# mikwieczorek/centroids-reid

Hardware: AMD Instinct MI355X
Metric: train_images_per_sec (higher is better)
Workload: dtype bf16; 1 GPU; ResNet50 256x128 CTL training step: fwd+bwd, centroid-triplet + center + xent, Adam + center SGD (BASELINE configs[1]); P=16, K=4, global_batch=64, num_classes=751, parallelism=single

## Files before the change

### centroids-reid_amd/_lib.py

```python
from __future__ import annotations

import ctypes as C
import os

import torch

_HERE = os.path.dirname(os.path.abspath(__file__))
LIB_PATH = os.environ.get("CREID_LIB_PATH") or os.path.join(_HERE, "lib", "libcreid_hip.so")

F32, BF16, F16 = 0, 1, 2
_DT = {torch.float32: F32, torch.bfloat16: BF16, torch.float16: F16}
BF16X3 = 3
EVAL_PRECISIONS = ("bf16x3",)
TRAIN_PRECISIONS = ("bf16x3",)

_lib = None

_p, _i64, _i32, _f32, _sz = C.c_void_p, C.c_int64, C.c_int32, C.c_float, C.c_size_t

SIGNATURES = {
    "creid_abi_version": (C.c_int, []),
    "creid_l2norm_rows": (C.c_int, [_p, _p, _p, _i64, _i64, C.c_int, _f32, _p]),
    "creid_row_sqnorm": (C.c_int, [_p, _p, _i64, _i64, C.c_int, _p]),
    "creid_sqdist_matrix": (C.c_int, [_p, _p, _p, _p, _i64, _i64, _i64, C.c_int, _p, _i64, _p]),
# ... 18 lines not shown
    "creid_stream_count_band_h16": (C.c_int, [_p, _p, _p, _p, _i64, _i64, _i64, C.c_int, _p, _p, _i32, _p, _p, _p, _p, _i32, _p, _p, _p,
                                              _p]),
    "creid_stream_count_rescore": (C.c_int, [_p, _p, _i64, _i32, _p, _p, _p, _p, _i64, _i64, _i32, _p, _p, _p, _p, _p, _p]),
    "creid_rerank_recip": (C.c_int, [_p, _i64, _i32, _i32, _p, _p, _p, _p]),
    "creid_rerank_weights": (C.c_int, [_p, _p, _p, _i64, _i64, _p, _p, _p, _p]),
    "creid_rerank_expand": (C.c_int, [_p, _i64, _i32, _i32, _p, _p, _p, _i32, _p, _p, _p, _p, _p]),
    "creid_rerank_blend": (C.c_int, [_p, _p, _i64, _i64, _f32, _p, _p, _p, _p, _p, _i32, _p, _p]),
    "creid_tune_set": (C.c_int, [_i32, _i64, _i64, _i64, _i64, _i32, _i32, _i32]),
    "creid_tune_clear": (C.c_int, []),
    "creid_tune_count": (_i64, [_i32, _i64, _i64, _i64, _i64, _i32]),
    "creid_loo_centroids_fwd": (C.c_int, [_p, _p, _i64, _i64, _i64, _p, _p, _p]),
    "creid_loo_centroids_bwd": (C.c_int, [_p, _p, _i64, _i64, _i64, _p, _p]),
    "creid_loo_emb_fwd": (C.c_int, [_p, _p, _p, _i64, _i64, _i64, _p, _p, _p, _p, _p, _p]),
    "creid_loo_emb_bwd": (C.c_int, [_p, _p, _i64, _i64, _i64, _p, _p]),
    "creid_ctl_step_stats": (C.c_int, [_p, _p, _i64, _i64, _p, _i64, _p, _p]),
    "creid_loo_emb_fwd_rows": (C.c_int, [_p, _p, _p, _i64, _i64, _i64, _p, _p, _p, _p, _p, _p, _p]),
    "creid_loo_emb_fwd_rows_lonely": (C.c_int, [_p, _p, _p, _i64, _i64, _i64, _p, _p, _p, _p, _p, _p, _p, _p]),
    "creid_triplet_fwd_batched_rows": (C.c_int, [_p, _p, _p, _i64, _i64, _i64, _f32, _i32, _p, _p, _p, _p, _p, _p, _p]),
    "creid_ctl_round_scale": (C.c_int, [_p, _i64, _p, _p]),
    "creid_ctl_heads_workspace_bytes": (_sz, [_i64, _i64, _i64, _i64, _i64]),
    "creid_ctl_heads_fused": (C.c_int, [_p, _p]),
    "creid_ctl_step_stats_rows": (C.c_int, [_p, _p, _i64, _i64, _i64, _p, _p, _p, _p]),
    "creid_center_loss_fwd_masked": (C.c_int, [_p, _p, _p, _p, _i64, _i64, _i64, _p, _p, _p]),
    "creid_center_loss_bwd_masked": (C.c_int, [_p, _p, _p, _p, _p, _i64, _i64, _p, _f32, _p, _p, _p]),
    "creid_xent_ls_masked": (C.c_int, [_p, _p, _p, _i64, _i64, _f32, _f32, _p, _p, _p, _p]),
    "creid_bn1d_fwd_masked": (C.c_int, [_p, _p, _i64, _i64, _p, _p, _p, _p, _f32, _f32, _p, _p, _p, _p]),
    "creid_bn1d_bwd_masked": (C.c_int, [_p, _p, _p, _i64, _i64, _p, _p, _p, _p, _p, _p, _p]),
    "creid_triplet_fwd": (C.c_int, [_p, _p, _p, _i64, _i64, _f32, _p, _p, _p, _p, _p, _p, _p, _p]),
    "creid_triplet_bwd": (C.c_int, [_p, _i64, _i64, _p, _p, _p, _p, _p, _p, _f32, _p, _p]),
    "creid_triplet_fwd_batched": (C.c_int, [_p, _p, _p, _i64, _i64, _i64, _f32, _p, _p, _p, _p, _p, _p, _p, _p]),
    "creid_triplet_bwd_batched": (C.c_int, [_p, _i64, _i64, _i64, _p, _p, _p, _p, _p, _p, _f32, _p, _p]),
    "creid_triplet_cosine_fwd": (C.c_int, [_p, _p, _p, _i64, _i64, _f32, _p, _p, _p, _p, _p, _p, _p, _p]),
    "creid_triplet_cosine_bwd": (C.c_int, [_p, _i64, _i64, _p, _p, _p, _p, _p, _p, _f32, _p, _p]),
    "creid_rownorm_fwd": (C.c_int, [_p, _i64, _i64, C.c_int, _f32, _p, _p, _p]),
    "creid_rownorm_bwd": (C.c_int, [_p, _p, _p, _i64, _i64, C.c_int, _f32, _p, _p]),
    "creid_hard_mine_from_dist": (C.c_int, [_p, _p, _i64, _p, _p, _p, _p, _p]),
    "creid_clamp_sqrt_inplace": (C.c_int, [_p, _i64, _f32, _p]),
    "creid_center_loss_fwd": (C.c_int, [_p, _p, _p, _i64, _i64, _i64, _p, _p, _p]),
    "creid_center_loss_bwd": (C.c_int, [_p, _p, _p, _p, _i64, _i64, _p, _f32, _p, _p, _p]),
    "creid_xent_ls": (C.c_int, [_p, _p, _i64, _i64, _f32, _f32, _p, _p, _p, _p]),
    "creid_bn1d_fwd": (C.c_int, [_p, _i64, _i64, _p, _p, _p, _p, C.c_int, _f32, _f32, _p, _p, _p, _p]),
    "creid_bn1d_bwd": (C.c_int, [_p, _p, _i64, _i64, _p, _p, _p, _p, _p, _p, _p]),
    "creid_gather_mean_rows": (C.c_int, [_p, _p, _p, _i64, _i64, _p, _p]),
    "creid_adam_step": (C.c_int, [_p, _p, _p, _p, _i64, _f32, _f32, _f32, _f32, _f32, _i64, _f32, _p]),
    "creid_adam_step_dev": (C.c_int, [_p, _p, _p, _p, _i64, _p, _f32, _f32, _f32, _f32, _f32, _p]),
    "creid_sgd_scaled_step": (C.c_int, [_p, _p, _i64, _f32, _f32, _p]),
    "creid_amp_scale": (C.c_int, [_p, _i64, _p, _p, _p]),
    "creid_amp_unscale_check": (C.c_int, [_p, _i64, _p, _p, _p]),
    "creid_amp_update": (C.c_int, [_p, _p, _f32, _f32, C.c_int32, _p]),
    "creid_adam_step_dev_amp": (C.c_int, [_p, _p, _p, _p, _i64, _p, _f32, _f32, _f32, _f32, _f32, _p, _p]),
    "creid_sgd_scaled_step_amp": (C.c_int, [_p, _p, _i64, _f32, _f32, _p, _p]),
    "creid_conv2d_bn_partial_rows": (_i64, [_p]),
    "creid_igemm_halo_launches": (_i64, []),
    "creid_wgrad_taps_launches": (_i64, []),
    "creid_conv2d_fwd_nhwc": (C.c_int, [_p, _p, _p, _p, _p, C.c_int, _p]),
    "creid_conv2d_fwd_affine_nhwc": (C.c_int, [_p, _p, _p, _p, _p, _p, C.c_int, C.c_int, _p]),
    "creid_conv1x1_bnrelu_fwd": (C.c_int, [_p, _p, _p, _i64, _i64, _i64, _p, _p, _p, _p, C.c_int, _p]),
    "creid_bn2d_fold_entry_bytes": (_i64, []),
    "creid_bn2d_fold_multi": (C.c_int, [_p, _i64, _p]),
    "creid_stem_conv_fwd_affine": (C.c_int, [_i64, _i64, _i64, _p, _p, _p, _p, C.c_int, C.c_int, _p]),
    "creid_stem_conv_pool_fwd_affine": (C.c_int, [_i64, _i64, _i64, _p, _p, _p, _p, C.c_int, C.c_int, _p]),
    "creid_bottleneck_c3_c1_fwd_affine": (C.c_int, [_i64, _i64, _i64, _i64, _p, _p, _p, _p, _p, _p, _p, _p, C.c_int, _p]),
    "creid_bottleneck_c3_c1_fwd_stats": (C.c_int, [_i64, _i64, _i64, _i64, _p, _p, _p, _p, _p, _p, _p, _p, C.c_int, _p]),
    "creid_conv2d_dgrad_nhwc": (C.c_int, [_p, _p, _p, _p, _p, C.c_int, _p]),
    "creid_conv2d_wgrad_workspace_bytes": (_sz, [_p, C.c_int]),
    "creid_conv2d_wgrad_nhwc": (C.c_int, [_p, _p, _p, _p, C.c_int, _p, _sz, C.c_int, _p]),
    "creid_conv2d_wgrad_partials": (C.c_int, [_p, _p, _p, _p, _sz, C.c_int, _p]),
    "creid_conv2d_wgrad_partials_bnfin": (C.c_int, [_p, _p, _p, _p, _sz, C.c_int, _p, _i64, _i64, _i64, _p, _p, _p, _p, _p, _p, _p]),
    "creid_conv2d_wgrad_reduce": (C.c_int, [_p, _p, C.c_int, _p, _sz, C.c_int, _p]),
    "creid_bn2d_bwd_finalize_wred": (C.c_int, [_p, _i64, _i64, _i64, _p, _p, _p, _p, _p, _p, _p, _p, C.c_int, _p, _sz, C.c_int, _p]),
    "creid_conv2d_wgrad_reduce_job": (C.c_int, [_p, _p, C.c_int, _p, _sz, C.c_int, _p]),
    "creid_conv2d_dgrad_x3_nhwc": (C.c_int, [_p, _p, _p, _p, _p, _p]),
    "creid_conv2d_wgrad_x3_workspace_bytes": (_sz, [_p]),
    "creid_conv2d_wgrad_x3_nhwc": (C.c_int, [_p, _p, _p, _p, C.c_int, _p, _sz, _p]),
    "creid_conv2d_wgrad_x3_partials": (C.c_int, [_p, _p, _p, _p, _sz, _p]),
    "creid_weight_prep_x3_train_multi": (C.c_int, [_p, _p, _i64, _i64, _p]),
    "creid_stem_conv_fwd": (C.c_int, [_i64, _i64, _i64, _p, _p, _p, _p, C.c_int, _p]),
    "creid_stem_conv_wgrad_workspace_bytes": (_sz, [_i64, _i64, _i64, C.c_int]),
    "creid_stem_conv_wgrad": (C.c_int, [_i64, _i64, _i64, _p, _p, _p, C.c_int, _p, _sz, C.c_int, _p]),
    "creid_image_to_nhwc4_pad": (C.c_int, [_p, _i64, _i64, _i64, C.c_int, _p, _p]),
    "creid_augment_u8": (C.c_int, [_p, _p, _i64, _i64, _i64, _i64] + [C.c_float] * 9 + [C.c_int32, C.c_int32, _p, _p]),
    "creid_resize_u8": (C.c_int, [_p, _i64, _p, _p, _p, _i64, _p, _i64, _i64, _i64, _p, _p]),
    "creid_weight_prep": (C.c_int, [_p, _i64, _i64, _i64, _i64, C.c_int, _p, _p, _p]),
    "creid_weight_prep_entry_bytes": (_i64, []),
    "creid_weight_prep_multi": (C.c_int, [_p, _p, _i64, _i64, C.c_int, _p]),
    "creid_stem_weight_prep": (C.c_int, [_p, C.c_int, _p, _p]),
    "creid_bn2d_finalize": (C.c_int, [_p, _i64, _i64, _i64, _p, _p, C.c_int, _f32, _f32, _p, _p, _p, _p, _p, _p]),
    "creid_col_stats_rows": (_i64, [_i64]),
    "creid_col_stats": (C.c_int, [_p, _i64, _i64, C.c_int, _p, _p]),
    "creid_bn2d_apply": (C.c_int, [_p, _p, _p, C.c_int, _i64, _i64, C.c_int, _p, _p]),
    "creid_bn2d_apply_mask": (C.c_int, [_p, _p, _p, C.c_int, _i64, _i64, C.c_int, _p, _p, _p]),
    "creid_bn2d_finalize_apply_mask": (C.c_int, [_p, _i64, _i64, _i64, _p, _p, _f32, _f32, _p, _p, _p, _p, _p, _p, _p, C.c_int, C.c_int, _p, _p, C.c_int, _p]),
    "creid_bn2d_apply_dual_mask": (C.c_int, [_p, _p, _p, _p, C.c_int, _i64, _i64, C.c_int, _p, _p, _p]),
    "creid_bn2d_bwd_rows": (_i64, [_i64]),
    "creid_bn2d_bwd": (C.c_int, [_p, _p, _p, _p, _p, _p, _i64, _i64, C.c_int, _p, C.c_int, _p, _p, _p, _p, _p, _p]),
    "creid_bn2d_bwd_mask": (C.c_int, [_p, _p, _p, _p, _p, _p, _p, _i64, _i64, C.c_int, _p, C.c_int, _p, _p, _p, _p, _p, _p]),
    "creid_bn2d_bwd_mask_reduce2": (C.c_int, [_p, _p, _p, _p, _p, _p, _i64, _i64, C.c_int, _p, C.c_int, _p, _p, _p, _p, _p, _p, _p, _p, _p]),
    "creid_conv2d_dgrad_bnred_nhwc": (C.c_int, [_p, _p, _p, _p, _p, _p, _p, _p, _p, _p, _i64, C.c_int, C.c_int, _p]),
    "creid_conv2d_dgrad_fused_nhwc": (C.c_int, [_p, _p, _p, _p, _p, C.c_int, _p, _p, _p, _p, _p, _p, _p, _i64, _p, _p, C.c_int, _p, _sz,
                                                C.c_int, _p]),
    "creid_ibn_rows_per_image": (_i64, [_i64]),
    "creid_ibn_fwd": (C.c_int, [_p, _i64, _i64, _i64, _i64, _p, _p, _p, _p, _p, _p, C.c_int, _f32, _f32, C.c_int, C.c_int,
                                _p, C.c_int, _p, _p, _p, _p, _p]),
    "creid_ibn_bwd": (C.c_int, [_p, _p, _p, _p, _p, _i64, _i64, _i64, _i64, _p, _p, C.c_int, _p, C.c_int, _p, _p, _p, _p, _p,
                                _p, _p, _p]),
    "creid_ibn_fwd_mask": (C.c_int, [_p, _i64, _i64, _i64, _i64, _p, _p, _p, _p, _p, _p, C.c_int, _f32, _f32, C.c_int, C.c_int, _p, C.c_int, _p, _p, _p, _p, _p, _p]),
# ... 106 lines not shown
```

### centroids-reid_amd/csrc/conv_igemm.hip

```cpp
#include "conv_epilogue.hpp"
#include <type_traits>
#include <atomic>
#include "wgrad_reduce.hpp"
#include "tune.hpp"
#include <stdlib.h>

bool wgrad_make_reduce_job(const creid_conv_desc* d, int dtype, const void* ws, size_t ws_bytes, float* dw, int accumulate,
                           WRedJob& j);
int wgrad_reduce_job_launch(const WRedJob& j, hipStream_t s);
int launch_stream1x1(int M, int K, int N, const void* src, const void* wgt, void* out, float* bn_part, hipStream_t s);
int launch_stream2(int M, int K, int N, const void* src, const void* wgt, void* out, float* bn_part, const void* add_src,
                   const float* epi_scale, const float* epi_shift, int epi_relu, int bn_cap, int dtype, hipStream_t s);
int launch_conv3x3_c64(int M, int H, int Wd, const void* src, const void* wgt, void* out, float* bn_part, const float* epi_scale,
                       const float* epi_shift, int epi_relu, int dtype, hipStream_t s);
int launch_igemm_pp(const IGemmGeom& g, const void* src, const void* wgt, void* out, const void* add_src, float* bn_part,
                    int variant, int dtype, hipStream_t s);

__device__ __attribute__((aligned(128))) unsigned g_zero_page[32];

template <int BN>
__global__ __launch_bounds__(256, BN == 128 ? 1 : 2) void igemm_bf16_kernel(IGemmGeom g, const unsigned short* __restrict__ src,
                                                         const unsigned short* __restrict__ wgt,
                                                         unsigned short* __restrict__ out,
                                                         const unsigned short* __restrict__ add_src,
// ... 811 lines not shown
    for (int tap = 0; tap < 9; ++tap) {
      const int dr = g.transposed ? 2 - tr : tr, dc = g.transposed ? 2 - ts : ts;
      int aoff[MI], kx[MI];
#pragma unroll
      for (int i = 0; i < MI; ++i) {
        const int hr = hr0[i] + dr, hc = hc0[i] + dc;
        aoff[i] = (hr * hp + hc) * BK;
        kx[i] = (((hc >> 1) + kmul * hr) & 7) ^ kh;
      }
      if (++ts == 3) { ts = 0; ++tr; }
#pragma unroll
      for (int kc = 0; kc < P; ++kc) {
        asm volatile("s_barrier" ::: "memory");
        const unsigned short* As = smem + kc * PLANE;
        const unsigned short* Bs = smem + HALO + buf * TILE_B;
        buf = (buf + 1 == NS) ? 0 : buf + 1;
        s16x8 a[2][MI], b[2][TNW];
        auto load_frags = [&](int kk, int sl) {
          const int ch = 2 * kk + kh;
#pragma unroll
          for (int i = 0; i < MI; ++i)
            a[sl][i] = *reinterpret_cast<const s16x8*>(&As[aoff[i] + (((2 * kk) ^ kx[i]) << 3)]);
#pragma unroll
          for (int j = 0; j < TNW; ++j) {
            const int c = wn * (BN / 2) + j * 32 + l31;
            b[sl][j] = *reinterpret_cast<const s16x8*>(&Bs[c * BK + ((ch ^ ((c >> 1) & 7)) << 3)]);
          }
        };
        auto mma = [&](int sl) {
          if (CREID_ABL_ON(g.abl, 1)) return;
#pragma unroll
          for (int i = 0; i < MI; ++i)
#pragma unroll
            for (int j = 0; j < TNW; ++j)
              acc[i][j] = ET::mfma(a[sl][i], b[sl][j], acc[i][j]);
        };
        load_frags(0, 0);
        __builtin_amdgcn_sched_barrier(0);
        load_frags(1, 1); mma(0);
        __builtin_amdgcn_sched_barrier(0);
        load_frags(2, 0); mma(1);
        __builtin_amdgcn_sched_barrier(0);
        load_frags(3, 1); mma(0);
        __builtin_amdgcn_sched_barrier(0);
        mma(1);
      }
    }
  }
  __syncthreads();

  igemm_tile_epilogue<ET, BM, BN, NT>(g, smem, acc, out, add_src, bn_part, bnred, tile_m, row0, col0, [](int rr) { return rr; });
}

template <int BN>
__global__ __launch_bounds__(256) void igemm_f32_kernel(IGemmGeom g, const float* __restrict__ src,
                                                        const float* __restrict__ wgt, float* __restrict__ out,
                                                        const float* __restrict__ add_src,
                                                        float* __restrict__ bn_part, int tiles_n) {
  constexpr int BK = 16, PA = 128 * 4 + 16, PB = BN * 4 + 16, TNW = BN / 64, NB = BN / 64;
  __shared__ __attribute__((aligned(16))) float As[2][2][2][PA];
  __shared__ __attribute__((aligned(16))) float Bs[2][2][2][PB];
  const int tid = threadIdx.x, lane = tid & 63, wave = tid >> 6;
  const int wm = wave >> 1, wn = wave & 1;
  const int bid = xcd_remap(blockIdx.x, gridDim.x);
  const int tile_m = bid / tiles_n, tile_n = bid % tiles_n;
  const int row0 = tile_m * 128, col0 = tile_n * BN;
  const int span_mask = (1 << g.log2span) - 1;

  const int lrow = tid >> 2, lkc = tid & 3;
  int oy[2], ox[2], bpix[2];
  bool vm[2];
#pragma unroll
  for (int i = 0; i < 2; ++i) {
    const int m = row0 + lrow + 64 * i;
    vm[i] = m < g.M;
    const int mm = vm[i] ? m : 0;
    const int b = mm / (g.OH * g.OW), rem = mm - b * (g.OH * g.OW);
    oy[i] = rem / g.OW; ox[i] = rem - oy[i] * g.OW;
    bpix[i] = b * g.SH * g.SW;
  }
  const float* wp[NB];
#pragma unroll
  for (int i = 0; i < NB; ++i) wp[i] = wgt + (int64_t)(col0 + lrow + 64 * i) * g.K + 4 * lkc;
  float4 ra[2], rb[NB];
  unsigned amask[2] = {0u, 0u};
  auto gload = [&](int t) {
    const int kk = t * BK + 4 * lkc;
    const int tap = kk >> g.log2span, c = kk & span_mask;
    const int r = tap / g.kw, s = tap - r * g.kw;
#pragma unroll
    for (int i = 0; i < 2; ++i) {
      int iy, ix;
      const bool ok = vm[i] && igemm_src_pixel(g, oy[i], ox[i], r, s, iy, ix);
      amask[i] = ok ? 0xffffffffu : 0u;
      const int64_t off = ok ? (int64_t)(bpix[i] + iy * g.SW + ix) * g.pitch + c : 0;
      ra[i] = *reinterpret_cast<const float4*>(src + off);
    }
#pragma unroll
    for (int i = 0; i < NB; ++i) rb[i] = *reinterpret_cast<const float4*>(wp[i] + t * BK);
  };
  const int sh = lkc >> 1, so = lrow * 4 + 2 * (lkc & 1);
  auto lstore = [&](int buf) {
#pragma unroll
    for (int i = 0; i < 2; ++i) {
      auto mk = [&](float v) { return __uint_as_float(__float_as_uint(v) & amask[i]); };
      *reinterpret_cast<float2*>(&As[buf][0][sh][so + 256 * i]) = make_float2(mk(ra[i].x), mk(ra[i].z));
// ... 77 lines not shown
    float s1 = 0.f, s2 = 0.f;
    const float esc = g.epi_scale ? g.epi_scale[c] : 1.f, esh = g.epi_scale ? g.epi_shift[c] : 0.f;
#pragma unroll
    for (int i = 0; i < 2; ++i) {
#pragma unroll
      for (int r = 0; r < 16; ++r) {
        const int rr = row0 + wm * 64 + i * 32 + (r & 3) + 8 * (r >> 2) + 4 * kh;
        if (rr < g.M) {
          float v = acc[i][j][r];
          if (g.epi_scale) v = fmaf(v, esc, esh);
          if (add_src) v += add_src[(int64_t)rr * g.N + c];
          if (g.epi_relu) v = fmaxf(v, 0.f);
          s1 += v; s2 = fmaf(v, v, s2);
          out[(int64_t)rr * g.N + c] = v;
        }
      }
    }
    if (bn_part) {
      s1 += __shfl_xor(s1, 32, 64); s2 += __shfl_xor(s2, 32, 64);
      if (kh == 0) { red[(wm * 2 + 0) * BN + cl] = s1; red[(wm * 2 + 1) * BN + cl] = s2; }
    }
  }
  if (bn_part) {
    __syncthreads();
    for (int i = tid; i < 2 * BN; i += 256) {
      const int which = i / BN, cl = i - which * BN;
      bn_part[((int64_t)tile_m * 2 + which) * g.N + col0 + cl] = red[(0 * 2 + which) * BN + cl] + red[(1 * 2 + which) * BN + cl];
    }
  }
}

static int use_dma_env() {
  static const int v = [] { const char* e = getenv("CREID_IGEMM_DMA"); return e ? atoi(e) : 1; }();
  return v;
}

static int ws_stages_env() {
  static const int v = [] { const char* e = getenv("CREID_IGEMM_WS_STAGES"); int x = e ? atoi(e) : 0; return (x == 2 || x == 4) ? x : 3; }();
  return v;
}

static bool igemm_halo_covers(const IGemmGeom& g, int bn, int stages) {
  const int c = 1 << g.log2span;
  if (g.kw != 3 || g.K != 9 * c || g.stride != 1 || g.pad != 1 || !g.check_bounds || g.parity || g.pitch != c) return false;
  if (c != 64 && c != 128 && c != 256) return false;
  if (g.SH != g.OH || g.SW != g.OW) return false;
  if (g.OW != 8 && g.OW != 16 && g.OW != 32 && g.OW != 64) return false;
  if ((g.OH * g.OW) % 128 != 0 || g.M % (g.OH * g.OW) != 0) return false;
  if ((128 / g.OW + 2) * (g.OW + 2) > 32 * halo_pw(c)) return false;
  if (stages < 2 || stages > 4 || (bn != 64 && bn != 128)) return false;
  return halo_lds_bytes(c, bn, stages) < 160 * 1024;
}
static std::atomic<long long> g_halo_launches{0};

static int launch_igemm(const IGemmGeom& g_in, const void* src, const void* wgt, void* out, const void* add_src,
                        float* bn_part, int dtype, hipStream_t s, BnRedArgs bnred = BnRedArgs{},
                        const WRedJob* wred_in = nullptr) {
#ifdef CREID_ABL_BUILD
  const char* abl_e = CREID_KNOB_ENV("CREID_IGEMM_ABL");
  const int abl_env = abl_e ? atoi(abl_e) : 0;
  { static int warned = -1; if (abl_env && abl_env != warned) { warned = abl_env; creid_ablation_env("CREID_IGEMM_ABL"); } }
#else
  const int abl_env = 0;
#endif
  if (!creid_is_storage(dtype)) return CREID_E_DTYPE;
  IGemmGeom g = g_in;
  g.abl = abl_env;
  WRedJob wred{};
  if (wred_in) wred = *wred_in;
  static_assert(sizeof(float) * (4 * 512 + 8192) <= 2 * (128 + 64) * 64 * 2, "reduce scratch must fit the smallest LDS ring");
  const int tiles_m = (g.M + 127) / 128;
  int bn = 128;
  static const int min_wgs = [] { const char* e = getenv("CREID_IGEMM_BN128_MIN_WGS"); int v = e ? atoi(e) : 0; return v > 0 ? v : 384; }();
  if (g.N % 128 != 0 || (int64_t)tiles_m * (g.N / 128) < min_wgs) bn = 64;
  TunePlan tp;
  int tuned_stages = 0, tuned_dma = 0, tuned_stream = 0, tuned_bm256 = 0, tuned_stream2 = 0, tuned_pp = -1;
  const int plan_d = g.transposed | (g.stride << 1);
  const bool plan_eval = creid_is16(dtype) && g.epi_scale && creid_tune_lookup(CREID_TUNE_IGEMM, g.M, g.N, g.K, plan_d | 8, tp);
  const bool have_plan = plan_eval || (creid_is16(dtype) && creid_tune_lookup(CREID_TUNE_IGEMM, g.M, g.N, g.K, plan_d, tp));
  int planned = -1;
  auto ran = [&](int kernel) {
    if (have_plan && kernel != planned) creid_tune_declined(CREID_TUNE_IGEMM, g.M, g.N, g.K, plan_eval ? (plan_d | 8) : plan_d);
  };
  if (have_plan && dtype == CREID_F16 && tp.p2 == 2) {
  } else if (have_plan && tp.p2 == 5) {
    tuned_pp = tp.p0;
    planned = 5;
  } else if (have_plan && (tp.p0 == 64 || tp.p0 == 128) && g.N % tp.p0 == 0 && (tp.p1 == 2 || tp.p1 == 3 || tp.p1 == 4)) {
    bn = tp.p0; tuned_stages = tp.p1; tuned_dma = tp.p2 == 1; tuned_stream = tp.p2 == 2; tuned_bm256 = tp.p2 == 3; tuned_stream2 = tp.p2 == 4;
    planned = (tp.p2 >= 1 && tp.p2 <= 4) ? tp.p2 : 0;
  }
  {
    const char* ce = CREID_KNOB_ENV("CREID_C64_3X3");
    const bool c64_on = !ce || atoi(ce) != 0;
    if (c64_on && creid_is16(dtype) && !g.transposed && g.N == 64 && g.K == 576 && g.log2span == 6 && g.kw == 3 && g.stride == 1 &&
        g.pad == 1 && g.pitch == 64 && g.check_bounds && !add_src && !bnred.x && !wred.ws && g.SH == g.OH && g.SW == g.OW &&
        !(bn_part && g.epi_scale)) {
      const int rc = launch_conv3x3_c64(g.M, g.OH, g.OW, src, wgt, out, bn_part, g.epi_scale, g.epi_shift, g.epi_relu, dtype, s);
      if (rc != CREID_E_SHAPE) { ran(6); return rc; }
    }
  }
  {
    const char* pe = CREID_KNOB_ENV("CREID_IGEMM_PP");
    const int force_pp = pe ? (int)strtol(pe, nullptr, 0) : 0;
    const bool pp_off = pe && force_pp == 0;
    if (creid_is16(dtype) && !bnred.x && !wred.ws && g.log2span >= 6 && !pp_off && (force_pp || tuned_pp >= 0)) {
// ... 36 lines not shown
      static const int parity_on = [] { const char* e = getenv("CREID_DGRAD_PARITY"); return e ? atoi(e) : 1; }();
      IGemmGeom gp = g;
      if (parity_on && g.transposed && g.stride == 2 && g.kw == 3 && g.pad == 1 && (g.K >> g.log2span) == 9 &&
          g.OH % 2 == 0 && g.OW % 2 == 0 && (g.M / 4) % 128 == 0 && !g.add_compact && bnred.tiles_per_image == 0)
        gp.parity = 1;
      int ws_stages = use_ws == 2 ? ws_stages_env() : ((bn == 64 && g.K >= ws_min_k) ? 3 : 2);
      if (tuned_stages && use_ws != 2) ws_stages = tuned_stages;
      const dim3 block_ws(512);
      {
        const char* be = CREID_KNOB_ENV("CREID_IGEMM_BM");
        const int force_bm = be ? atoi(be) : 0;
        static const int bm256_min = [] { const char* e = getenv("CREID_IGEMM_BM256_MIN_WGS"); int v = e ? atoi(e) : 0; return v > 0 ? v : 256; }();
        const bool can256 = g.N % 128 == 0 && !bnred.x && !gp.parity;
        const int64_t wgs256 = (int64_t)((g.M + 255) / 256) * (g.N / 128);
        if (can256 && force_bm != 128 && (tuned_bm256 || (force_bm == 256 && wgs256 >= bm256_min))) {
          const int st256 = (ws_stages >= 3 || g.K >= 256) ? 3 : 2;
          const dim3 grid256((unsigned)(wgs256 + (wred.ws ? wred.nblocks : 0)));
          const int tn256 = g.N / 128;
#define CREID_WS256_LAUNCH(NS_, ET_)                                                                                  \
  hipLaunchKernelGGL((igemm_bf16_ws_kernel<128, NS_, 256, ET_>), grid256, block_ws, 0, s, gp, (const unsigned short*)src, \
                     (const unsigned short*)wgt, (unsigned short*)out, (const unsigned short*)add_src, bn_part, tn256, bnred, wred)
          if (dtype == CREID_F16) { if (st256 == 3) CREID_WS256_LAUNCH(3, F16T); else CREID_WS256_LAUNCH(2, F16T); }
          else { if (st256 == 3) CREID_WS256_LAUNCH(3, Bf16T); else CREID_WS256_LAUNCH(2, Bf16T); }
#undef CREID_WS256_LAUNCH
          ran(tuned_bm256 ? 3 : -2);
          return (int)hipGetLastError();
        }
      }
      if (ws_stages == 4 && bn == 128 && !(tuned_stages == 4 && use_ws != 2)) ws_stages = 3;
      const dim3 grid_ws((unsigned)(tiles_m * tiles_n + (wred.ws ? wred.nblocks : 0)));
      {
        const char* he = CREID_KNOB_ENV("CREID_IGEMM_HALO");
        if ((!he || atoi(he) != 0) && igemm_halo_covers(gp, bn, ws_stages)) {
          const int hc = 1 << gp.log2span;
#define CREID_HALO_LAUNCH1(C_, BN_, NS_, ET_)                                                                             \
  hipLaunchKernelGGL((igemm_bf16_halo_kernel<C_, BN_, NS_, ET_>), grid_ws, block_ws, 0, s, gp, (const unsigned short*)src, \
                     (const unsigned short*)wgt, (unsigned short*)out, (const unsigned short*)add_src, bn_part, tiles_n,  \
                     bnred, wred)
#define CREID_HALO_LAUNCH(C_, BN_, NS_) do { if (dtype == CREID_F16) CREID_HALO_LAUNCH1(C_, BN_, NS_, F16T); else CREID_HALO_LAUNCH1(C_, BN_, NS_, Bf16T); } while (0)
#define CREID_HALO_STAGES(C_, BN_) do { constexpr int NS4 = halo_lds_bytes(C_, BN_, 4) < 160 * 1024 ? 4 : 3;            \
                                        if (ws_stages == 4) CREID_HALO_LAUNCH(C_, BN_, NS4);                            \
                                        else if (ws_stages == 2) CREID_HALO_LAUNCH(C_, BN_, 2); else CREID_HALO_LAUNCH(C_, BN_, 3); } while (0)
#define CREID_HALO_BN(C_) do { if (bn == 128) CREID_HALO_STAGES(C_, 128); else CREID_HALO_STAGES(C_, 64); } while (0)
          if (hc == 64) CREID_HALO_BN(64); else if (hc == 128) CREID_HALO_BN(128); else CREID_HALO_BN(256);
#undef CREID_HALO_BN
#undef CREID_HALO_STAGES
#undef CREID_HALO_LAUNCH
#undef CREID_HALO_LAUNCH1
          g_halo_launches.fetch_add(1, std::memory_order_relaxed);
          ran(0);
          return (int)hipGetLastError();
        }
      }
#define CREID_WS_LAUNCH1(BN_, NS_, ET_)                                                                               \
  hipLaunchKernelGGL((igemm_bf16_ws_kernel<BN_, NS_, 128, ET_>), grid_ws, block_ws, 0, s, gp, (const unsigned short*)src, \
                     (const unsigned short*)wgt, (unsigned short*)out, (const unsigned short*)add_src, bn_part, tiles_n, \
                     bnred, wred)
#define CREID_WS_LAUNCH(BN_, NS_) do { if (dtype == CREID_F16) CREID_WS_LAUNCH1(BN_, NS_, F16T); else CREID_WS_LAUNCH1(BN_, NS_, Bf16T); } while (0)
      if (bn == 128) { if (ws_stages == 4) CREID_WS_LAUNCH(128, 4); else if (ws_stages == 2) CREID_WS_LAUNCH(128, 2); else CREID_WS_LAUNCH(128, 3); }
      else { if (ws_stages == 4) CREID_WS_LAUNCH(64, 4); else if (ws_stages == 2) CREID_WS_LAUNCH(64, 2); else CREID_WS_LAUNCH(64, 3); }
#undef CREID_WS_LAUNCH
#undef CREID_WS_LAUNCH1
      ran(0);
      return (int)hipGetLastError();
    }
    if (wred.ws) { const int rc = wgrad_reduce_job_launch(wred, s); if (rc) return rc; wred.ws = nullptr; }
    static const int stages_env = [] { const char* e = getenv("CREID_IGEMM_STAGES"); int v = e ? atoi(e) : 0; return (v >= 2 && v <= 5) ? v : 2; }();
    const int stages = (tuned_dma && tuned_stages) ? tuned_stages : stages_env;
#define CREID_DMA_LAUNCH1(BN_, NS_, ET_)                                                                               \
  hipLaunchKernelGGL((igemm_bf16_dma_kernel<BN_, NS_, ET_>), grid, block, 0, s, g, (const unsigned short*)src,         \
                     (const unsigned short*)wgt, (unsigned short*)out, (const unsigned short*)add_src, bn_part, tiles_n, \
                     bnred)
#define CREID_DMA_LAUNCH(BN_, NS_) do { if (dtype == CREID_F16) CREID_DMA_LAUNCH1(BN_, NS_, F16T); else CREID_DMA_LAUNCH1(BN_, NS_, Bf16T); } while (0)
    if (bn == 128) {
      switch (stages) { case 2: CREID_DMA_LAUNCH(128, 2); break; case 3: CREID_DMA_LAUNCH(128, 3); break;
                        case 4: case 5: CREID_DMA_LAUNCH(128, 4); break;
                        default: CREID_DMA_LAUNCH(128, 2); break; }
    } else {
      switch (stages) { case 2: CREID_DMA_LAUNCH(64, 2); break; case 3: CREID_DMA_LAUNCH(64, 3); break;
                        case 4: CREID_DMA_LAUNCH(64, 4); break; case 5: CREID_DMA_LAUNCH(64, 5); break;
                        default: CREID_DMA_LAUNCH(64, 2); break; }
    }
#undef CREID_DMA_LAUNCH
#undef CREID_DMA_LAUNCH1
    ran(1);
    return (int)hipGetLastError();
  } else if (bnred.x || g.add_mask || (g.epi_scale && creid_is16(dtype)) || dtype == CREID_F16) {
    return CREID_E_DTYPE;
  } else if (wred.ws && wgrad_reduce_job_launch(wred, s) != 0) {
    return (int)hipGetLastError();
  } else if (dtype == CREID_BF16) {
    if (g.K % 64 != 0) return CREID_E_SHAPE;
    if (bn == 128)
      hipLaunchKernelGGL(igemm_bf16_kernel<128>, grid, block, 0, s, g, (const unsigned short*)src,
                         (const unsigned short*)wgt, (unsigned short*)out, (const unsigned short*)add_src, bn_part, tiles_n);
    else
      hipLaunchKernelGGL(igemm_bf16_kernel<64>, grid, block, 0, s, g, (const unsigned short*)src,
                         (const unsigned short*)wgt, (unsigned short*)out, (const unsigned short*)add_src, bn_part, tiles_n);
  } else if (dtype == CREID_F32) {
    if (g.K % 16 != 0) return CREID_E_SHAPE;
    if (bn == 128)
      hipLaunchKernelGGL(igemm_f32_kernel<128>, grid, block, 0, s, g, (const float*)src, (const float*)wgt, (float*)out,
                         (const float*)add_src, bn_part, tiles_n);
    else
      hipLaunchKernelGGL(igemm_f32_kernel<64>, grid, block, 0, s, g, (const float*)src, (const float*)wgt, (float*)out,
                         (const float*)add_src, bn_part, tiles_n);
  } else {
    return CREID_E_DTYPE;
  }
  ran(-2);
  return (int)hipGetLastError();
}

static int check_desc(const creid_conv_desc* d) {
  if (!d || d->batch <= 0 || d->in_h <= 0 || d->in_w <= 0 || d->in_c <= 0 || d->out_c <= 0) return CREID_E_ARG;
  if (d->kh != d->kw || (d->kh != 1 && d->kh != 3) || d->stride < 1 || d->stride > 2) return CREID_E_SHAPE;
  if (igemm_ilog2(d->in_c) < 0 || igemm_ilog2(d->out_c) < 0 || d->in_c < 64 || d->out_c < 64) return CREID_E_SHAPE;
  if (d->out_h != (d->in_h + 2 * d->pad - d->kh) / d->stride + 1) return CREID_E_SHAPE;
  if (d->out_w != (d->in_w + 2 * d->pad - d->kw) / d->stride + 1) return CREID_E_SHAPE;
  if (d->batch * d->in_h * d->in_w >= (1LL << 24) || d->batch * d->out_h * d->out_w >= (1LL << 24) || d->batch * d->in_h * d->in_w * d->in_c > (1LL << 40)) return CREID_E_SHAPE;
  return 0;
}

int conv_check_desc(const creid_conv_desc* d) { return check_desc(d); }

extern "C" {

int64_t creid_igemm_halo_launches(void) { return (int64_t)g_halo_launches.load(std::memory_order_relaxed); }

int64_t creid_conv2d_bn_partial_rows(const creid_conv_desc* d) {
  if (!d) return 0;
  return (d->batch * d->out_h * d->out_w + 127) / 128;
}

int creid_conv2d_fwd_nhwc(const creid_conv_desc* d, const void* x, const void* w_krsc, void* y, float* bn_partial,
                          int dtype, void* stream) {
  int rc = check_desc(d);
  if (rc) return rc;
  CREID_CHECK_ARG(x && w_krsc && y);
  IGemmGeom g = fwd_geom(d);
  if (dtype == CREID_BF16X3) return launch_igemm_x3(g, x, w_krsc, y, nullptr, bn_partial, as_stream(stream));
  return launch_igemm(g, x, w_krsc, y, nullptr, bn_partial, dtype, as_stream(stream));
}

int creid_conv2d_fwd_affine_nhwc(const creid_conv_desc* d, const void* x, const void* w_krsc, void* y, const float* scale_shift,
                                 const void* residual, int relu, int dtype, void* stream) {
  int rc = check_desc(d);
  if (rc) return rc;
  CREID_CHECK_ARG(x && w_krsc && y && scale_shift);
  IGemmGeom g = fwd_geom(d);
  g.epi_scale = scale_shift; g.epi_shift = scale_shift + d->out_c; g.epi_relu = relu ? 1 : 0;
  if (dtype == CREID_BF16X3) return launch_igemm_x3(g, x, w_krsc, y, residual, nullptr, as_stream(stream));
  return launch_igemm(g, x, w_krsc, y, residual, nullptr, dtype, as_stream(stream));
}

int creid_conv2d_dgrad_nhwc(const creid_conv_desc* d, const void* dy, const void* w_crsk, void* dx, const void* add_src,
                            int dtype, void* stream) {
  int rc = check_desc(d);
  if (rc) return rc;
  CREID_CHECK_ARG(dy && w_crsk && dx);
  IGemmGeom g = dgrad_geom(d);
  return launch_igemm(g, dy, w_crsk, dx, add_src, nullptr, dtype, as_stream(stream));
}

int creid_conv2d_dgrad_x3_nhwc(const creid_conv_desc* d, const void* dy, const void* w2_crsk, void* dx, const void* add_src,
                               void* stream) {
  int rc = check_desc(d);
  if (rc) return rc;
  CREID_CHECK_ARG(dy && w2_crsk && dx);
  IGemmGeom g = dgrad_geom(d);
  return launch_igemm_x3(g, dy, w2_crsk, dx, add_src, nullptr, as_stream(stream));
}

int creid_conv2d_dgrad_bnred_nhwc(const creid_conv_desc* d, const void* dy, const void* w_crsk, void* dx,
                                  const void* add_src, const void* bn_x, const void* bn_act, const float* bn_mean,
                                  const float* bn_invstd, float* bn_partial, int64_t bn_stat_image_rows,
                                  int add_src_stride, int dtype, void* stream) {
  int rc = check_desc(d);
  if (rc) return rc;
  CREID_CHECK_ARG(dy && w_crsk && dx && bn_x && bn_mean && bn_invstd && bn_partial && bn_stat_image_rows >= 0);
  return creid_conv2d_dgrad_fused_nhwc(d, dy, w_crsk, dx, add_src, add_src_stride, nullptr, bn_x, bn_act, nullptr, bn_mean, bn_invstd,
// ... 53 lines not shown
```

### include/creid.h

```cpp
#ifndef CREID_H
#define CREID_H

#include <stddef.h>
#include <stdint.h>

#ifdef __cplusplus
extern "C" {
#endif

#define CREID_ABI_VERSION 1

enum { CREID_F32 = 0, CREID_BF16 = 1, CREID_F16 = 2, CREID_BF16X3 = 3 };
enum { CREID_E_ARG = -1, CREID_E_DTYPE = -2, CREID_E_WS = -3, CREID_E_SHAPE = -4 };

int creid_abi_version(void);


int creid_l2norm_rows(const float* x, void* y, float* sqnorm, int64_t rows, int64_t D,
                      int out_dtype, float eps, void* stream);

int creid_row_sqnorm(const void* x, float* out, int64_t rows, int64_t D, int dtype, void* stream);

int creid_sqdist_matrix(const void* q, const void* g, const float* qq, const float* gg,
                        int64_t m, int64_t n, int64_t D, int dtype, float* out, int64_t ldo,
// ... 192 lines not shown
                              float* dist_an, int32_t* p_idx, int32_t* n_idx, void* stream);

int creid_clamp_sqrt_inplace(float* d, int64_t n, float lo, void* stream);

int creid_center_loss_fwd(const float* x, const int64_t* labels, const float* centers, int64_t B,
                          int64_t C, int64_t D, float* row_sq, float* loss, void* stream);
int creid_center_loss_bwd(const float* x, const int64_t* labels, const float* centers,
                          const float* row_sq, int64_t B, int64_t D, const float* gscale_dev,
                          float gscale, float* dx_accum, float* dcenters_accum, void* stream);

int creid_xent_ls(const float* logits, const int64_t* targets, int64_t B, int64_t C, float eps,
                  float gscale, float* row_loss, float* loss, float* dlogits, void* stream);

int creid_bn1d_fwd(const float* x, int64_t B, int64_t D, const float* weight, const float* bias,
                   float* running_mean, float* running_var, int training, float momentum, float eps,
                   float* y, float* save_mean, float* save_invstd, void* stream);
int creid_bn1d_bwd(const float* x, const float* dy, int64_t B, int64_t D, const float* weight,
                   const float* save_mean, const float* save_invstd, float* dx_accum,
                   float* dweight_accum, float* dbias_accum, void* stream);

int creid_gather_mean_rows(const float* emb, const int64_t* order, const int64_t* offsets,
                           int64_t n_seg, int64_t D, float* out, void* stream);


int creid_adam_step(float* p, const float* g, float* m, float* v, int64_t n, float lr, float beta1,
                    float beta2, float eps, float weight_decay, int64_t step, float grad_scale,
                    void* stream);
int creid_adam_step_dev(float* p, const float* g, float* m, float* v, int64_t n, float* hyper_dev,
                        float beta1, float beta2, float eps, float weight_decay, float grad_scale,
                        void* stream);
int creid_sgd_scaled_step(float* p, float* g, int64_t n, float lr, float grad_mul, void* stream);

int creid_amp_scale(const float* x, int64_t n, const float* amp_state, float* y, void* stream);
int creid_amp_unscale_check(float* g, int64_t n, const float* amp_state, int32_t* amp_flags, void* stream);
int creid_amp_update(float* amp_state, int32_t* amp_flags, float growth_factor, float backoff_factor, int32_t growth_interval,
                     void* stream);
int creid_adam_step_dev_amp(float* p, const float* g, float* m, float* v, int64_t n, float* hyper_dev, float beta1, float beta2,
                            float eps, float weight_decay, float grad_scale, const int32_t* skip_flag, void* stream);
int creid_sgd_scaled_step_amp(float* p, float* g, int64_t n, float lr, float grad_mul, const int32_t* skip_flag, void* stream);


int creid_gemm_f32(const float* A, int64_t sam, int64_t sak, const float* B, int64_t sbk, int64_t sbn,
                   float* C, int64_t ldc, int64_t M, int64_t N, int64_t K, float alpha, float beta,
                   int32_t split_k, void* stream);


typedef struct {
  int64_t batch, in_h, in_w, in_c, out_h, out_w, out_c;
  int32_t kh, kw, stride, pad;
} creid_conv_desc;

int64_t creid_conv2d_bn_partial_rows(const creid_conv_desc* d);
int64_t creid_igemm_halo_launches(void);
int64_t creid_wgrad_taps_launches(void);
int creid_conv2d_fwd_nhwc(const creid_conv_desc* d, const void* x, const void* w_krsc, void* y,
                          float* bn_partial, int dtype, void* stream);
int creid_conv2d_fwd_affine_nhwc(const creid_conv_desc* d, const void* x, const void* w_krsc, void* y,
                                 const float* scale_shift, const void* residual, int relu, int dtype, void* stream);
int creid_conv1x1_bnrelu_fwd(const void* x_raw, const float* scale_shift, const void* w_krsc, int64_t M, int64_t K, int64_t N,
                             void* y, float* bn_partial, void* a_out, uint8_t* mask_out, int dtype, void* stream);
int64_t creid_bn2d_fold_entry_bytes(void);
int creid_bn2d_fold_multi(const void* table_dev, int64_t n_entries, void* stream);
int creid_conv2d_dgrad_nhwc(const creid_conv_desc* d, const void* dy, const void* w_crsk, void* dx,
                            const void* add_src, int dtype, void* stream);
int creid_conv2d_dgrad_x3_nhwc(const creid_conv_desc* d, const void* dy, const void* w2_crsk, void* dx, const void* add_src,
                               void* stream);
int creid_conv2d_dgrad_bnred_nhwc(const creid_conv_desc* d, const void* dy, const void* w_crsk, void* dx,
                                  const void* add_src, const void* bn_x, const void* bn_act,
                                  const float* bn_mean, const float* bn_invstd, float* bn_partial,
                                  int64_t bn_stat_image_rows, int add_src_stride, int dtype, void* stream);

int creid_conv2d_dgrad_fused_nhwc(const creid_conv_desc* d, const void* dy, const void* w_crsk, void* dx,
                                  const void* add_src, int add_src_stride, const uint8_t* add_mask, const void* bn_x,
                                  const void* bn_act, const uint8_t* bn_mask, const float* bn_mean, const float* bn_invstd,
                                  float* bn_partial, int64_t bn_stat_image_rows, const creid_conv_desc* wred_desc, float* wred_dw,
                                  int wred_accumulate, const void* wred_ws, size_t wred_ws_bytes, int dtype,
                                  void* stream);
size_t creid_conv2d_wgrad_workspace_bytes(const creid_conv_desc* d, int dtype);
int creid_conv2d_wgrad_nhwc(const creid_conv_desc* d, const void* x, const void* dy, float* dw_oihw,
                            int accumulate, void* ws, size_t ws_bytes, int dtype, void* stream);
int creid_conv2d_wgrad_partials(const creid_conv_desc* d, const void* x, const void* dy, void* ws,
                                size_t ws_bytes, int dtype, void* stream);
int creid_bn2d_bwd_finalize_wred(const float* bn_partial, int64_t bn_rows, int64_t bn_C, int64_t bn_count,
                                 const float* bn_mean, const float* bn_invstd, const float* bn_gamma, float* bn_sums,
                                 float* bn_dgamma, float* bn_dbeta, const creid_conv_desc* wred_desc, float* wred_dw,
                                 int wred_accumulate, const void* wred_ws, size_t wred_ws_bytes, int dtype, void* stream);
int creid_conv2d_wgrad_reduce_job(const creid_conv_desc* d, float* dw_oihw, int accumulate, const void* ws,
                                  size_t ws_bytes, int dtype, void* stream);
size_t creid_conv2d_wgrad_x3_workspace_bytes(const creid_conv_desc* d);
int creid_conv2d_wgrad_x3_nhwc(const creid_conv_desc* d, const void* x, const void* dy, float* dw_oihw, int accumulate,
                               void* ws, size_t ws_bytes, void* stream);
int creid_conv2d_wgrad_x3_partials(const creid_conv_desc* d, const void* x, const void* dy, void* ws, size_t ws_bytes,
                                   void* stream);
int creid_conv2d_wgrad_partials_bnfin(const creid_conv_desc* d, const void* x, const void* dy, void* ws, size_t ws_bytes,
                                      int dtype, const float* bn_partial, int64_t bn_rows, int64_t bn_C, int64_t bn_count,
                                      const float* bn_mean, const float* bn_invstd, const float* bn_gamma, float* bn_sums,
                                      float* bn_dgamma, float* bn_dbeta, void* stream);
int creid_conv2d_wgrad_reduce(const creid_conv_desc* d, float* dw_oihw, int accumulate, const void* ws,
                              size_t ws_bytes, int dtype, void* stream);

int creid_stem_conv_fwd(int64_t batch, int64_t H, int64_t W, const void* xpad, const void* w_stem, void* y,
                        float* bn_partial, int dtype, void* stream);
int creid_stem_conv_fwd_affine(int64_t batch, int64_t H, int64_t W, const void* xpad, const void* w_stem, void* y,
                               const float* scale_shift, int relu, int dtype, void* stream);
int creid_stem_conv_pool_fwd_affine(int64_t batch, int64_t H, int64_t W, const void* xpad, const void* w_stem, void* y,
                                    const float* scale_shift, int relu, int dtype, void* stream);
// ... 96 lines not shown
```

Baseline: 11180 images/s.

## Add whole-image LDS-resident implicit-GEMM kernel for 512-channel 3x3 convs

Adds a warp-specialized implicit-GEMM kernel for stride-1 3x3 convolutions with 512 channels on 128-pixel feature maps. The whole input image tile (all channel planes) is loaded once into LDS, and all 9 taps are computed from it by shifting addresses with zero masking, while producer waves stream weights through a ring buffer. This avoids reloading shifted input tiles per tap. The kernel is enabled by default when the geometry matches and can be disabled via an env knob. It uses a large LDS footprint and relies on hand-counted vmcnt waits.

```diff
diff --git a/centroids-reid_amd/_lib.py b/centroids-reid_amd/_lib.py
--- a/centroids-reid_amd/_lib.py
+++ b/centroids-reid_amd/_lib.py
@@ -94,6 +94,7 @@
     "creid_sgd_scaled_step_amp": (C.c_int, [_p, _p, _i64, _f32, _f32, _p, _p]),
     "creid_conv2d_bn_partial_rows": (_i64, [_p]),
     "creid_igemm_halo_launches": (_i64, []),
+    "creid_igemm_image_launches": (_i64, []),
     "creid_wgrad_taps_launches": (_i64, []),
     "creid_conv2d_fwd_nhwc": (C.c_int, [_p, _p, _p, _p, _p, C.c_int, _p]),
     "creid_conv2d_fwd_affine_nhwc": (C.c_int, [_p, _p, _p, _p, _p, _p, C.c_int, C.c_int, _p]),
diff --git a/centroids-reid_amd/csrc/conv_igemm.hip b/centroids-reid_amd/csrc/conv_igemm.hip
--- a/centroids-reid_amd/csrc/conv_igemm.hip
+++ b/centroids-reid_amd/csrc/conv_igemm.hip
@@ -887,6 +887,201 @@
   igemm_tile_epilogue<ET, BM, BN, NT>(g, smem, acc, out, add_src, bn_part, bnred, tile_m, row0, col0, [](int rr) { return rr; });
 }
 
+constexpr int image_lds_bytes(int C, int BN, int NS) { return ((C / 64) * 128 * 64 + NS * BN * 64) * 2; }
+
+template <int C, int BN, int NS, typename ET = Bf16T>
+__global__ __launch_bounds__(512, 1) void igemm_bf16_image_kernel(IGemmGeom g, const unsigned short* __restrict__ src,
+                                                                  const unsigned short* __restrict__ wgt,
+                                                                  unsigned short* __restrict__ out,
+                                                                  const unsigned short* __restrict__ add_src,
+                                                                  float* __restrict__ bn_part, int tiles_n,
+                                                                  BnRedArgs bnred, WRedJob wred) {
+  constexpr int NT = 512, BM = 128;
+  constexpr int BK = 64, TNW = BN / 64, NBI = BN / 32, MI = 2;
+  constexpr int P = C / 64, PW = 4;
+  constexpr int PLANE = BM * BK, IMAGE = P * PLANE;
+  constexpr int TILE_B = BN * BK;
+  constexpr int LDS_ELEMS = IMAGE + NS * TILE_B;
+  static_assert(C == 512, "channels per tap");
+  static_assert(NS >= 2 && NS <= 4, "ring depth");
+  static_assert(LDS_ELEMS * 2 == image_lds_bytes(C, BN, NS) && LDS_ELEMS * 2 <= 160 * 1024, "image + weight ring must fit the LDS");
+  static_assert(BN * (BM + 4) <= LDS_ELEMS && (NT / (BN / 8)) * 2 * BN * 2 <= LDS_ELEMS, "C staging and column-sum scratch of the epilogue");
+  static_assert(sizeof(float) * (4 * 512 + 8192) <= LDS_ELEMS * 2, "reduce scratch of the piggy-backed job");
+  constexpr int D = 3;
+  static_assert(P >= 3 && (9 * P) % D == 0 && (D + 1) * NBI + 2 * PW <= 63, "vmcnt is a 6-bit counter");
+  __shared__ __attribute__((aligned(1024))) unsigned short smem[LDS_ELEMS];
+  const int tid = threadIdx.x, lane = tid & 63, wave = tid >> 6;
+  const int nred = wred.ws ? wred.nblocks : 0;
+  const int ntile_wgs = (int)gridDim.x - nred;
+  if ((int)blockIdx.x >= ntile_wgs) {
+    wgrad_reduce_block<NT>(wred, (int)blockIdx.x - ntile_wgs, reinterpret_cast<float*>(smem));
+    return;
+  }
+  const bool producer = wave >= 4;
+  const int cw = wave & 3;
+  const int wm = cw >> 1, wn = cw & 1;
+  const int bid = xcd_remap((int)blockIdx.x, ntile_wgs);
+  const int tile_m = bid / tiles_n, tile_n = bid % tiles_n;
+  const int row0 = tile_m * BM, col0 = tile_n * BN;
+  const int l31 = lane & 31, kh = lane >> 5;
+  const int log2ow = 31 - __clz(g.OW);
+  const int kmul = g.OW == 8 ? 4 : 0;
+  constexpr int nk = 9 * P;
+
+  f32x16 acc[MI][TNW];
+  if (producer) {
+    const int lr8 = lane >> 3, lcp = lane & 7;
+    typedef const void __attribute__((address_space(1)))* gptr_t;
+    typedef void __attribute__((address_space(3)))* lptr_t;
+    const unsigned short* iptr[PW];
+#pragma unroll
+    for (int j = 0; j < PW; ++j) {
+      const int slot = (j * 4 + cw) * 8 + lr8;
+      const int key = (((slot & (g.OW - 1)) >> 1) + kmul * (slot >> log2ow)) & 7;
+      iptr[j] = src + (int64_t)(row0 + slot) * g.pitch + ((lcp ^ key) << 3);
+    }
+    auto plane = [&](int p) {
+#pragma unroll
+      for (int j = 0; j < PW; ++j) {
+        __builtin_amdgcn_global_load_lds((gptr_t)iptr[j], (lptr_t)(smem + p * PLANE + (j * 4 + cw) * 512), 16, 0, 0);
+        iptr[j] += BK;
+      }
+    };
+    const unsigned short* wp[NBI];
+#pragma unroll
+    for (int i = 0; i < NBI; ++i) {
+      const int r = (i * 4 + cw) * 8 + lr8;
+      wp[i] = wgt + (int64_t)(col0 + r) * g.K + ((lcp ^ ((r >> 1) & 7)) << 3);
+    }
+    typedef unsigned u32x4 __attribute__((ext_vector_type(4)));
+    u32x4 wr0[NBI], wr1[NBI], wr2[NBI];
+    auto wload = [&](u32x4 (&r)[NBI]) {
+#pragma unroll
+      for (int i = 0; i < NBI; ++i) {
+        asm volatile("global_load_dwordx4 %0, %1, off" : "=v"(r[i]) : "v"(wp[i]) : "memory");
+        wp[i] += BK;
+      }
+    };
+    auto wstore = [&](const u32x4 (&r)[NBI], int buf) {
+      unsigned short* lb = smem + IMAGE + buf * TILE_B + cw * 512 + lane * 8;
+#pragma unroll
+      for (int i = 0; i < NBI; ++i) *reinterpret_cast<u32x4*>(lb + i * 2048) = r[i];
+    };
+    constexpr int LAST = nk - NS - D;
+    int buf = 0;
+    auto step = [&](int t, u32x4 (&r)[NBI]) {
+      if (t + NS - 1 < nk) {
+        const int younger = t < 0 ? 0 : min(D - 1, max(0, LAST - (t - D + 1) + 1));
+        if (younger >= 2) wait_vm<2 * NBI>();
+        else if (younger == 1) wait_vm<NBI>();
+        else wait_vm<0>();
+        wstore(r, buf);
+      }
+      buf = (buf + 1 == NS) ? 0 : buf + 1;
+      __builtin_amdgcn_sched_barrier(0);
+      if (t + 2 < P) plane(t + 2);
+      __builtin_amdgcn_sched_barrier(0);
+      if (t <= LAST) wload(r);
+      __builtin_amdgcn_sched_barrier(0);
+      if (t >= 0 && t + 2 < P) wait_vm<2 * NBI + PW>();
+      else if (t >= 0 && t + 1 < P) wait_vm<2 * NBI>();
+      if (t + 1 < nk) asm volatile("s_waitcnt lgkmcnt(0)\n\ts_barrier" ::: "memory");
+    };
+    static_assert(D == 3, "the waits above count D - 1 = 2 steps");
+    plane(0);
+    __builtin_amdgcn_sched_barrier(0);
+    wload(wr0); wload(wr1); wload(wr2);
+    if constexpr (NS == 2) {
+      step(-1, wr0);
+      for (int t0 = 0; t0 < nk; t0 += D) { step(t0, wr1); step(t0 + 1, wr2); step(t0 + 2, wr0); }
+    } else if constexpr (NS == 3) {
+      wait_vm<0>(); wstore(wr0, buf++); wload(wr0);
+      step(-1, wr1);
+      for (int t0 = 0; t0 < nk; t0 += D) { step(t0, wr2); step(t0 + 1, wr0); step(t0 + 2, wr1); }
+    } else {
+      wait_vm<0>(); wstore(wr0, buf++); wload(wr0);
+      wstore(wr1, buf++); wload(wr1);
+      step(-1, wr2);
+      for (int t0 = 0; t0 < nk; t0 += D) { step(t0, wr0); step(t0 + 1, wr1); step(t0 + 2, wr2); }
+    }
+  } else {
+#pragma unroll
+    for (int i = 0; i < MI; ++i)
+#pragma unroll
+      for (int j = 0; j < TNW; ++j)
+#pragma unroll
+        for (int r = 0; r < 16; ++r) acc[i][j][r] = 0.f;
+    const int oh = BM >> log2ow;
+    int y0[MI], x0[MI];
+#pragma unroll
+    for (int i = 0; i < MI; ++i) {
+      const int r = wm * (BM / 2) + i * 32 + l31;
+      y0[i] = r >> log2ow; x0[i] = r & (g.OW - 1);
+    }
+    int buf = 0, tr = 0, ts = 0;
+    for (int tap = 0; tap < 9; ++tap) {
+      const int dr = g.transposed ? 2 - tr : tr, dc = g.transposed ? 2 - ts : ts;
+      int aoff[MI], kx[MI];
+      bool inside[MI];
+#pragma unroll
+      for (int i = 0; i < MI; ++i) {
+        const int py = y0[i] + dr - 1, px = x0[i] + dc - 1;
+        inside[i] = (unsigned)py < (unsigned)oh && (unsigned)px < (unsigned)g.OW;
+        const int wy = py & (oh - 1), wx = px & (g.OW - 1);
+        aoff[i] = ((wy << log2ow) + wx) * BK;
+        kx[i] = (((wx >> 1) + kmul * wy) & 7) ^ kh;
+      }
+      if (++ts == 3) { ts = 0; ++tr; }
+#pragma unroll
+      for (int kc = 0; kc < P; ++kc) {
+        asm volatile("s_waitcnt lgkmcnt(0)\n\ts_barrier" ::: "memory");
+        const unsigned short* As = smem + kc * PLANE;
+        const unsigned short* Bs = smem + IMAGE + buf * TILE_B;
+        buf = (buf + 1 == NS) ? 0 : buf + 1;
+        s16x8 a[2][MI], b[2][TNW];
+        auto load_frags = [&](int kk, int sl) {
+          const int ch = 2 * kk + kh;
+#pragma unroll
+          for (int i = 0; i < MI; ++i)
+            a[sl][i] = *reinterpret_cast<const s16x8*>(&As[aoff[i] + (((2 * kk) ^ kx[i]) << 3)]);
+#pragma unroll
+          for (int j = 0; j < TNW; ++j) {
+            const int c = wn * (BN / 2) + j * 32 + l31;
+            b[sl][j] = *reinterpret_cast<const s16x8*>(&Bs[c * BK + ((ch ^ ((c >> 1) & 7)) << 3)]);
+          }
+        };
+        auto mma = [&](int sl) {
+          if (CREID_ABL_ON(g.abl, 1)) return;
+#pragma unroll
+          for (int i = 0; i < MI; ++i) {
+            const s16x8 az = inside[i] ? a[sl][i] : s16x8(0);
+#pragma unroll
+            for (int j = 0; j < TNW; ++j)
+              acc[i][j] = ET::mfma(az, b[sl][j], acc[i][j]);
+          }
+        };
+        auto order = [&]() {
+          __builtin_amdgcn_sched_group_barrier(0x100, MI + TNW, 0);
+          __builtin_amdgcn_sched_group_barrier(0x002, 4 * MI, 0);
+          __builtin_amdgcn_sched_group_barrier(0x008, MI * TNW, 0);
+        };
+        load_frags(0, 0);
+        __builtin_amdgcn_sched_barrier(0);
+        load_frags(1, 1); mma(0); order();
+        __builtin_amdgcn_sched_barrier(0);
+        load_frags(2, 0); mma(1); order();
+        __builtin_amdgcn_sched_barrier(0);
+        load_frags(3, 1); mma(0); order();
+        __builtin_amdgcn_sched_barrier(0);
+        mma(1);
+      }
+    }
+  }
+  __syncthreads();
+
+  igemm_tile_epilogue<ET, BM, BN, NT>(g, smem, acc, out, add_src, bn_part, bnred, tile_m, row0, col0, [](int rr) { return rr; });
+}
+
 template <int BN>
 __global__ __launch_bounds__(256) void igemm_f32_kernel(IGemmGeom g, const float* __restrict__ src,
                                                         const float* __restrict__ wgt, float* __restrict__ out,
@@ -1070,6 +1265,18 @@
   return halo_lds_bytes(c, bn, stages) < 160 * 1024;
 }
 static std::atomic<long long> g_halo_launches{0};
+
+static bool igemm_image_covers(const IGemmGeom& g, int bn, int stages) {
+  const int c = 1 << g.log2span;
+  if (g.kw != 3 || g.K != 9 * c || g.stride != 1 || g.pad != 1 || !g.check_bounds || g.parity || g.pitch != c) return false;
+  if (c != 512) return false;
+  if (g.SH != g.OH || g.SW != g.OW) return false;
+  if (g.OH * g.OW != 128 || (g.OW != 8 && g.OW != 16)) return false;
+  if (g.M % 128 != 0) return false;
+  if (stages < 2 || stages > 4 || (bn != 64 && bn != 128)) return false;
+  return image_lds_bytes(c, bn, bn == 128 ? 2 : stages) <= 160 * 1024;
+}
+static std::atomic<long long> g_image_launches{0};
 
 static int launch_igemm(const IGemmGeom& g_in, const void* src, const void* wgt, void* out, const void* add_src,
                         float* bn_part, int dtype, hipStream_t s, BnRedArgs bnred = BnRedArgs{},
@@ -1212,6 +1419,25 @@
           return (int)hipGetLastError();
         }
       }
+      {
+        const char* ie = CREID_KNOB_ENV("CREID_IGEMM_IMAGE");
+        if ((!ie || atoi(ie) != 0) && igemm_image_covers(gp, bn, ws_stages)) {
+#define CREID_IMAGE_LAUNCH1(BN_, NS_, ET_)                                                                                \
+  hipLaunchKernelGGL((igemm_bf16_image_kernel<512, BN_, NS_, ET_>), grid_ws, block_ws, 0, s, gp, (const unsigned short*)src, \
+                     (const unsigned short*)wgt, (unsigned short*)out, (const unsigned short*)add_src, bn_part, tiles_n,  \
+                     bnred, wred)
+#define CREID_IMAGE_LAUNCH(BN_, NS_) do { if (dtype == CREID_F16) CREID_IMAGE_LAUNCH1(BN_, NS_, F16T); else CREID_IMAGE_LAUNCH1(BN_, NS_, Bf16T); } while (0)
+          if (bn == 128) CREID_IMAGE_LAUNCH(128, 2);
+          else if (ws_stages == 4) CREID_IMAGE_LAUNCH(64, 4);
+          else if (ws_stages == 2) CREID_IMAGE_LAUNCH(64, 2);
+          else CREID_IMAGE_LAUNCH(64, 3);
+#undef CREID_IMAGE_LAUNCH
+#undef CREID_IMAGE_LAUNCH1
+          g_image_launches.fetch_add(1, std::memory_order_relaxed);
+          ran(0);
+          return (int)hipGetLastError();
+        }
+      }
 #define CREID_WS_LAUNCH1(BN_, NS_, ET_)                                                                               \
   hipLaunchKernelGGL((igemm_bf16_ws_kernel<BN_, NS_, 128, ET_>), grid_ws, block_ws, 0, s, gp, (const unsigned short*)src, \
                      (const unsigned short*)wgt, (unsigned short*)out, (const unsigned short*)add_src, bn_part, tiles_n, \
@@ -1287,6 +1513,7 @@
 extern "C" {
 
 int64_t creid_igemm_halo_launches(void) { return (int64_t)g_halo_launches.load(std::memory_order_relaxed); }
+int64_t creid_igemm_image_launches(void) { return (int64_t)g_image_launches.load(std::memory_order_relaxed); }
 
 int64_t creid_conv2d_bn_partial_rows(const creid_conv_desc* d) {
   if (!d) return 0;
diff --git a/include/creid.h b/include/creid.h
--- a/include/creid.h
+++ b/include/creid.h
@@ -268,6 +268,7 @@
 
 int64_t creid_conv2d_bn_partial_rows(const creid_conv_desc* d);
 int64_t creid_igemm_halo_launches(void);
+int64_t creid_igemm_image_launches(void);
 int64_t creid_wgrad_taps_launches(void);
 int creid_conv2d_fwd_nhwc(const creid_conv_desc* d, const void* x, const void* w_krsc, void* y,
                           float* bn_partial, int dtype, void* stream);
```

New measurement: 11290 images/s (median of 6 runs). About the same (+0.9%).
